# richarddurbin/modimizer

Measured on AMD Instinct MI355X. Metric: Gbp/s hashed+sketched (k=21,d=64), higher is better.
Workload: dtype u64; 1 GPU; BASELINE config 2: 10 Gbp synthetic ONT-like reads (log-normal N50 20 kb, 5% subs, 30x of a 333 Mbp genome), k=21 d=64 seed=17, seqhash scan + modset build (table bits 30); reads_per_gpu=598835, bases_per_gpu=10000000000, modimizers_per_gpu=156043826, modset_entries=102967436, k=21, d=64, table_bits=30, parallelism=reads sharded x1, modset per GPU

## Files before the change

modimizer_amd/csrc/mg_bucket.hip:

```cpp
#include "mg_table.h"



template <bool PACKED>
__device__ __forceinline__ void mgOccurrence (const MgBucketArgs &a, U32 b, U64 x, U32 t, U64 *m, U32 *ord)
{
  if (PACKED)
    { *ord = (U32) (x & (((U64) 1 << a.f.ordBits) - 1));
      *m = ((U64) (b >> a.f.loB) << a.f.remBits) | (x >> a.f.ordBits);
    }
  else { *m = x; *ord = t; }
}

__device__ __forceinline__ void mgDedupCount (const MgBucketArgs &a, U32 *sOrd, U32 *sCnt, U32 at, U32 ord)
{
  const U32 tok = mgToken (ord);
  if (a.markDup)
    { const U32 old = atomicMax (&sOrd[at], tok);
      const U32 loser = old > tok ? tok : old;
      if (loser MG_ABLATE_AND (!(a.debug & 1))) a.flags[0x7fffffffu - loser] = 0;
    }
  else atomicMax (&sOrd[at], tok);
  atomicAdd (&sCnt[at], 1u);
}
// ... 189 lines not shown
  const U32 R = a.g.R, T = blockDim.x, tid = threadIdx.x;
  unsigned long long *sKey = reinterpret_cast<unsigned long long *> (mgDynLds);
  U32 *sOrd = reinterpret_cast<U32 *> (mgDynLds + (size_t) R * 8);
  U32 *sCnt = sOrd + R;
  U32 *sGrp = sCnt + R;
  const U32 nGrp = a.nSlices + 1;
  U32 b = blockIdx.x * bucketsPerBlock, bEnd = b + bucketsPerBlock;
  U64 hotAt = blockIdx.x; const U64 nHot = HOT ? a.hotCount[1] : 0;
  if (HOT) { if (hotAt >= nHot) return; }
  else
    { if (bEnd > a.nBuckets) bEnd = a.nBuckets;
      if (b >= bEnd) return;
    }
  for (U32 i = tid ; i < R ; i += T) { sKey[i] = 0; sOrd[i] = 0; sCnt[i] = 0; }
  if (tid < MG_RANK_GROUPS) sGrp[tid] = 0;
  for ( ; ; )
  {
  if (HOT) { b = a.hotBuckets[hotAt]; bEnd = b + 1; }
  U64 lo = a.bucketStart[b], hi = a.bucketStart[b + 1];
  U32 occNow = a.occ[b];
  U64 ck[MG_BUCKET_PREFETCH]; U32 ct[MG_BUCKET_PREFETCH];
#pragma unroll
  for (int j = 0 ; j < MG_BUCKET_PREFETCH ; ++j)
    { U64 i = lo + (U64) j * T + tid; ck[j] = 0; ct[j] = 0; if (!HOT && i < hi) { ck[j] = __builtin_nontemporal_load (&a.pK[i]); if (!PACKED) ct[j] = __builtin_nontemporal_load (&a.pT[i]); } }
  __syncthreads ();
  for ( ; b < bEnd ; ++b)
    {
      U64 nlo = hi, nhi = hi;
      U64 nk[MG_BUCKET_PREFETCH]; U32 nt[MG_BUCKET_PREFETCH];
#pragma unroll
// ... 47 lines not shown
              rk[j] = 0; rc[j] = 0; ro[j] = 0; rp[j] = 0;
              if (i < R) rk[j] = sKey[i];
              if (rk[j])
                { rc[j] = sCnt[i]; ro[j] = sOrd[i];
                  sKey[i] = 0; sOrd[i] = 0; sCnt[i] = 0;
                  rk[j] = (rk[j] - 1) | (SLOT ? (unsigned long long) i << MG_SLOT_SHIFT : 0ull);
                  if (rc[j]) rp[j] = atomicAdd (&sGrp[mgIsAssigned (ro[j]) ? a.nSlices : ((0x7fffffffu - ro[j]) >> a.sliceShift)], 1u);
                }
            }
          __syncthreads ();
          const int lane = (int) (tid & 63);
          const U32 gv = (U32) lane < nGrp ? sGrp[lane] : 0;
          const U32 gIncl = mgWaveInclusiveSum (gv);
          const U32 gBase = gIncl - gv;
          const U32 total = (U32) __builtin_amdgcn_readlane ((int) gIncl, 63);
          if (tid < 64)
            { if ((U32) lane <= nGrp) a.sliceOff[(U64) b * (nGrp + 1) + lane] = (unsigned short) gBase;
              if (lane == 0) a.uniqCount[b] = total;
            }
#pragma unroll
          for (int j = 0 ; j < PER ; ++j)
            { const U32 grp = mgIsAssigned (ro[j]) ? a.nSlices : ((0x7fffffffu - ro[j]) >> a.sliceShift);
              const U32 at = (U32) __shfl ((int) gBase, (int) (rc[j] ? grp : 0)) + rp[j];
              if (rc[j]) { sKey[at] = rk[j]; sOrd[at] = ro[j]; sCnt[at] = rc[j]; }
            }
          __syncthreads ();
          if (tid < MG_RANK_GROUPS) sGrp[tid] = 0;
          for (U32 i = tid ; i < total ; i += T)
            { const U64 k = sKey[i]; const U32 ord = sOrd[i], c = sCnt[i];
              sKey[i] = 0; sOrd[i] = 0; sCnt[i] = 0;
              if (true MG_ABLATE_AND (!(a.debug & 8)))
                { __builtin_nontemporal_store (k, &a.pK[lo + i]); __builtin_nontemporal_store (ord, &a.pT[lo + i]); __builtin_nontemporal_store (c, &a.pC[lo + i]); }
              if (!a.markDup && !mgIsAssigned (ord) MG_ABLATE_AND (!(a.debug & 1))) a.flags[0x7fffffffu - ord] = 1;
            }
          __syncthreads ();
        }
      lo = nlo; hi = nhi; occNow = occNext;
#pragma unroll
      for (int j = 0 ; j < MG_BUCKET_PREFETCH ; ++j) { ck[j] = nk[j]; ct[j] = nt[j]; }
    }
  if (!HOT) break;
  hotAt += gridDim.x;
  if (hotAt >= nHot) break;
  }
}

__device__ __forceinline__ U32 mgPlaceStarts (U32 *cnt, unsigned short *sStart, int *sWave, U32 R, U32 T, U32 tid, U32 n)
{
  const U32 per = (R + 4 * T - 1) / (4 * T) * 4;
  const U32 j0 = tid * per, j1 = j0 + per < R ? j0 + per : R;
  U32 vS = 0; int vM = 0;
  for (U32 j = j0 ; j < j1 ; j += 4)
    { const uint4 c = *reinterpret_cast<const uint4 *> (&cnt[j]);
      int m = (int) j - (int) vS;               vM = m > vM ? m : vM; vS += c.x;
      m = (int) (j + 1) - (int) vS;             vM = m > vM ? m : vM; vS += c.y;
      m = (int) (j + 2) - (int) vS;             vM = m > vM ? m : vM; vS += c.z;
      m = (int) (j + 3) - (int) vS;             vM = m > vM ? m : vM; vS += c.w;
    }
  const int lane = (int) (tid & 63);
// ... 245 lines not shown
{
  unsigned long long sum = 0; U32 mx = 0;
  for (U32 b = blockIdx.x * 256 + threadIdx.x ; b < nBuckets ; b += gridDim.x * 256) { const U32 c = uniqCount[b]; sum += c; mx = c > mx ? c : mx; }
  sum = mgWaveReduce<MgSum> ((U64) sum); mx = mgWaveReduce<MgMax> (mx);
  if ((threadIdx.x & 63) == 0) { if (sum) atomicAdd (&out[0], sum); if (mx) atomicMax (&out[1], (unsigned long long) mx); }
}


MgStatus mgBucketDedup (const MgBucketArgs &a, bool packed, unsigned threads, unsigned grid, U32 perBlock, size_t lds, hipStream_t st)
{
  const U32 R = a.g.R;
  const bool bigR = R > MG_DEDUP_PER * 1024u;
  if (R > MG_DEDUP_PER_BIG * 1024u) { mgSetError ("internal: bucket of %u slots", R); return MG_ERR_ARG; }
  if ((U64) threads * (bigR ? MG_DEDUP_PER_BIG : MG_DEDUP_PER) < R)
    { mgSetError ("internal: %u threads for a bucket of %u slots", threads, R); return MG_ERR_ARG; }
  MG_HIP (hipMemsetAsync (a.hotCount, 0, 16, st));
  MG_LAUNCH (MG_K_HOT_REDUCE, st, mgHotPlanKernel, dim3 ((a.nBuckets + 255) / 256), dim3 (256), 0, st, a);
  const size_t ldsHot = (size_t) R * 16 + 16;
  const MgStatus s = mgForFlag (packed, [&] (auto PK) -> MgStatus
    { if (ldsHot > 48 * 1024) MG_HIP (hipFuncSetAttribute ((const void *) mgHotReduceKernel<decltype (PK)::value>, hipFuncAttributeMaxDynamicSharedMemorySize, (int) ldsHot));
      MG_LAUNCH (MG_K_HOT_REDUCE, st, mgHotReduceKernel<decltype (PK)::value>, dim3 (1024), dim3 (threads), ldsHot, st, a);
      return MG_OK;
    });
  if (s) return s;
  return mgForFlag (packed, [&] (auto PK) -> MgStatus { return mgForFlag (a.slotShift != 0, [&] (auto SL) -> MgStatus { return mgForFlag (bigR, [&] (auto BIG) -> MgStatus
    { constexpr bool pk = decltype (PK)::value, sl = decltype (SL)::value;
      constexpr int per = decltype (BIG)::value ? MG_DEDUP_PER_BIG : MG_DEDUP_PER;
      if (lds > 48 * 1024)
        { MG_HIP (hipFuncSetAttribute ((const void *) mgBucketDedupKernel<pk, sl, per, false>, hipFuncAttributeMaxDynamicSharedMemorySize, (int) lds));
          MG_HIP (hipFuncSetAttribute ((const void *) mgBucketDedupKernel<pk, sl, per, true>, hipFuncAttributeMaxDynamicSharedMemorySize, (int) lds));
        }
// ... 32 lines not shown
```

modimizer_amd/csrc/mg_common.h:

```cpp
#ifndef MG_COMMON_H
#define MG_COMMON_H
#include "mg_knobs.h"

#include <hip/hip_runtime.h>
#include <stdint.h>
#include <time.h>
#include <algorithm>
#include <vector>
#include "modgpu.h"

#define MG_WAVE 64

#define MG_SCAN_THREADS   256
#define MG_POS_PER_THREAD 64
#define MG_TILE_BASES     (64 * MG_POS_PER_THREAD)
#define MG_TILE_WORDS     (MG_TILE_BASES / 16)

struct MgHashParams {
  U64 factor1;
  U64 mask;
  int k;
  int shift1;
  U32 d;
  int dShift;
// ... 189 lines not shown
  U16 *baseDepth;
  bool baseZero;
  U64 *liveHist;
  bool liveHistValid;
  U32 size;
  U32 max;
  U32 syncedMax;
  U64 *counters;
  bool pendingDepth;
  bool dirty;
  U64 *find8;
  U64 find8Cap;
  U64 find8Version, version;
  bool empty;
  U64 *pin;
  int newPct;
  int loadPct;
  int  maxLog2Slots;
  U32  wantR;
  U64  diag[7];
  int  tightPct;
};
MgStatus mgTableAlloc (MgTable *t, U64 slotsWanted, hipStream_t st);
MgStatus mgTableEnsure (MgTable *t, U64 nIncoming, hipStream_t st);
MgStatus mgTableRollback (MgTable *t, hipStream_t st);
MgStatus mgTableClean (MgTable *t, hipStream_t st);
void     mgTableForget (MgTable *t, hipStream_t st);
size_t   mgTableAddScratchBytes (const MgTable *t, U64 n);
bool     mgTableUseBuckets (const MgTable *t, U64 n);
MgStatus mgTableAdd (MgTable *t, const U64 *dKmer, U64 n, int withDepth, void *scratch, hipStream_t st,
// ... 32 lines not shown
```

modimizer_amd/csrc/mg_knobs.c:

```c
#define _GNU_SOURCE
#include <pthread.h>
#include <sched.h>
#include <stdio.h>
#include <stdlib.h>
#include <string.h>
#include <unistd.h>
#include <sys/mman.h>
#include "mg_knobs.h"

static MgKnobs gKnobs;
static pthread_once_t gOnce = PTHREAD_ONCE_INIT;

static long num (const char *name)
{ const char *e = getenv (name); return e && *e ? atol (e) : MG_KNOB_UNSET; }

static void readAll (void)
{
  MgKnobs k;
  const char *e = getenv ("MODGPU_TABLE_PATH");
  k.tablePath = e && *e ? (long) e[0] : MG_KNOB_UNSET;
  e = getenv ("MODGPU_FIND_PATH");
  k.findPath = e && *e ? (long) e[0] : MG_KNOB_UNSET;
  k.partPacked = num ("MODGPU_PART_PACKED");       k.partBig = num ("MODGPU_PART_BIG");
  k.addChunk = num ("MODGPU_ADD_CHUNK");           k.scanGrid = num ("MODGPU_SCAN_GRID");
  k.scanGeneric = num ("MODGPU_SCAN_GENERIC");     k.scanHist = num ("MODGPU_SCAN_HIST");
  k.scanDiv64 = num ("MODGPU_SCAN_DIV64");        k.minTiled = num ("MODGPU_MIN_TILED");
  k.minTile = num ("MODGPU_MIN_TILE");
  k.noSegmentInput = num ("MODGPU_NO_SEGMENT_INPUT");
  k.rankSliceShift = num ("MODGPU_RANK_SLICE_SHIFT");
  k.flagPolarity = num ("MODGPU_FLAG_POLARITY");   k.mergeSlots = num ("MODGPU_MERGE_SLOTS");
  k.mergePlace = num ("MODGPU_MERGE_PLACE");
  k.bucketR = num ("MODGPU_BUCKET_R");             k.bucketT = num ("MODGPU_BUCKET_T");
  e = getenv ("MODGPU_HOT_SPLIT");
  k.hotSplit = e && *e ? atol (e) : MG_KNOB_UNSET;
  { const char *c = e ? strchr (e, ',') : 0; k.hotChunk = c ? atol (c + 1) : MG_KNOB_UNSET; }
  k.noAvx2 = num ("MODGPU_NO_AVX2");               k.textHost = num ("MODGPU_TEXT_HOST");
  k.textWindowKb = num ("MODGPU_TEXT_WINDOW_KB");   k.bgzfHost = num ("MODGPU_BGZF_HOST");
// ... 61 lines not shown
```

modimizer_amd/csrc/mg_knobs.h:

```cpp
#ifndef MG_KNOBS_H
#define MG_KNOBS_H
#include <limits.h>
#ifdef __cplusplus
extern "C" {
#endif
#define MG_KNOB_UNSET LONG_MIN
typedef struct {
  long findPath;
  long tablePath;
  long partPacked;
  long partBig;
  long addChunk;
  long scanGrid;
  long scanGeneric;
  long minTile;
  long minTiled;
  long scanDiv64;
  long scanHist;
  long noSegmentInput;
  long rankSliceShift;
  long flagPolarity;
  long mergeSlots;
  long mergePlace;
  long bucketR, bucketT;
  long hotSplit, hotChunk;
  long noAvx2;
  long textHost;
  long textWindowKb;
  long fileBatchMbp;
  long fileBatchBases;
  long readsetHost;
  long overlapCands;
  long testModsBatch;
  long overlapLds;
  long bgzfHost;
  long textIdsDevice;
  long gzipHost;
  long gzipChunkKb;
  long gzipBatch;
  long gzipRatio;
// ... 32 lines not shown
```

modimizer_amd/csrc/mg_modsetdev.hip:

```cpp
#include <unordered_map>
#include "mg_api_int.h"
#include "mg_xfer.h"

struct MgOnDevice
{ int before = -1; bool moved = false;
  explicit MgOnDevice (int dev) { if (dev >= 0 && hipGetDevice (&before) == hipSuccess && before != dev) moved = hipSetDevice (dev) == hipSuccess; }
  ~MgOnDevice () { if (moved) (void) hipSetDevice (before); }
};

static std::mutex gRegLock;
static std::unordered_map<const Modset *, MgDev *> gReg;
extern "C" { volatile int mgLiveDeviceModsets = 0; }

MgDev *mgDevLookup (const Modset *ms)
{ std::lock_guard<std::mutex> g (gRegLock); auto it = gReg.find (ms); return it == gReg.end () ? 0 : it->second; }

static void mgDevFree (MgDev *d)
{
  if (!d) return;
  MgOnDevice here (d->device);
  if (d->hPin) (void) hipHostFree (d->hPin);
  if (d->built)
    { (void) hipFree (d->t.slots); (void) hipFree (d->t.value); (void) hipFree (d->t.occ); (void) hipFree (d->t.find8);
      (void) hipFree (d->t.baseDepth); (void) hipFree (d->t.counters); (void) hipFree (d->t.liveHist);
    }
  if (d->side) { (void) hipStreamSynchronize (d->side); (void) hipStreamDestroy (d->side); }
  d->arena.release (); d->arena2.release ();
  for (int i = 0 ; i < 2 ; ++i) if (d->scanned[i]) (void) hipEventDestroy (d->scanned[i]);
  if (d->inputReady) (void) hipEventDestroy (d->inputReady);
  delete d;
}

static void mgDevDrop (Modset *ms, MgDev *d)
{
  { std::lock_guard<std::mutex> g (gRegLock); gReg.erase (ms); mgLiveDeviceModsets = (int) gReg.size (); }
  mgDevFree (d);
}

static MgStatus mgDevOnCallersGpu (const MgDev *d, bool quiet = false)
// ... 16 lines not shown
  MgTable &t = d->t;
  if (ms->tableBits < 20 || ms->tableBits > 32)
    { mgSetError ("device modset supports table bits 20..32 (got %d)", ms->tableBits); return MG_ERR_ARG; }
  memset (&t, 0, sizeof (t));
  t.maxLog2Slots = ms->tableBits - 1;
  t.kbits = 2 * ms->hasher->k;
  t.wantR = 4096;
  { const long r = mgKnobs ()->bucketR; if (r != MG_KNOB_UNSET && r >= 256) t.wantR = (U32) r; }
  t.size = ms->size;
  t.pin = d->hPin + 24;
  U64 cap = (ms->tableSize >> 2);
  MG_HIP (hipMalloc ((void **) &t.value, cap * sizeof (U64)));
  MG_HIP (hipMalloc ((void **) &t.baseDepth, cap * sizeof (U16)));
  MG_HIP (hipMalloc ((void **) &t.counters, 64));
  d->built = true;
  MG_HIP (hipMemsetAsync (t.baseDepth, 0, cap * sizeof (U16), st));
  MG_HIP (hipMemsetAsync (t.counters, 0, 64, st));
  { MgStatus s0 = mgTableEnsure (&t, ms->max, st); if (s0) return s0; }
  t.max = 0; t.syncedMax = 0;
  t.baseZero = !ms->max;
  if (ms->max)
    { MG_HIP (hipStreamSynchronize (st));
      MgStatus s;
      if ((s = mgXferH2D (t.value, ms->value, ((size_t) ms->max + 1) * sizeof (U64)))) return s;
      if ((s = mgXferH2D (t.baseDepth, ms->depth, ((size_t) ms->max + 1) * sizeof (U16)))) return s;
      if ((s = mgTableLoadHost (&t, t.value, 1, ms->max, st))) return s;
      MG_HIP (hipStreamSynchronize (st));
      t.max = t.syncedMax = ms->max;
    }
  d->hostIndexMax = ms->max;
// ... 194 lines not shown


U64 mgAddChunkSize (void)
{
  const long c = mgKnobs ()->addChunk;
  U64 v = c != MG_KNOB_UNSET && c > 0 ? (U64) c : ((U64) 1 << 30);
  if (v > ((U64) 1 << 30)) v = (U64) 1 << 30;
  return v;
}

static MgStatus mgAddChunk (Modset *ms, MgDev *d, const U64 *dKmer, U64 n, U32 *dIndexOut, int withDepth,
                            void *scratch, hipStream_t st, const MgHistReq *counted = 0, const MgSegSrc *segSrc = 0)
{
  MgTable &t = d->t;
  MgStatus s;
  MG_HIP (hipMemsetAsync (t.counters, 0, 16, st));
  if ((s = mgTableAdd (&t, dKmer, n, withDepth, scratch, st, counted, segSrc))) return s;
  volatile U64 *c = d->hPin;
  MG_HIP (hipMemcpyAsync (d->hPin, t.counters, 16, hipMemcpyDeviceToHost, st));
  MG_HIP (hipStreamSynchronize (st));
  U64 newMax = (U64) t.max + c[0];
  if (c[1] || newMax >= t.size)
    {
      if ((s = mgTableRollback (&t, st))) return s;
      mgSetError ("hashTableSize %u is too small for %llu", t.size, (unsigned long long) newMax);
      return MG_ERR_CAPACITY;
    }
  t.max = (U32) newMax;
  ms->max = t.max;
  if (n >= 4096) t.newPct = (int) (c[0] * 100 / n);
  if (dIndexOut && (s = mgTableFind (&t, dKmer, n, dIndexOut, st))) return s;
// ... 145 lines not shown
```

modimizer_amd/csrc/mg_part.hip:

```cpp
#include "mg_table.h"


__global__ void mgSubSegKernel (const MgSegSrc src, U64 n, U32 sub, MgSubSeg *__restrict__ subSeg)
{
  const U64 q = (U64) blockIdx.x * blockDim.x + threadIdx.x;
  if (q * sub >= n) return;
  const U32 w = mgSegOfOrdinal (src, q * sub);
  MgSubSeg e; e.w = w; e.s0 = src.segStart[w]; e.s1 = src.segStart[w + 1];
  subSeg[q] = e;
}

__global__ __launch_bounds__ (MG_PART_MAXBINS)
void mgPartChunksKernel (const U64 *__restrict__ segStart, U32 nSeg, U32 chunkElems, U32 *__restrict__ chunkBase)
{
  __shared__ U32 sS[MG_PART_MAXBINS];
  const U32 t = threadIdx.x;
  U32 c = t < nSeg ? (U32) ((segStart[t + 1] - segStart[t] + chunkElems - 1) / chunkElems) : 0;
  sS[t] = c;
  __syncthreads ();
  for (int off = 1 ; off < MG_PART_MAXBINS ; off <<= 1)
    { U32 v = t >= (U32) off ? sS[t - off] : 0;
      __syncthreads ();
      sS[t] += v;
      __syncthreads ();
// ... 252 lines not shown
      c = nc; seg = nseg; lo = nlo; hi = nhi; sub = nsub; have = nhave;
    }
}


MgStatus mgPartPass (const MgTable *t, MgPartPassArgs &p, hipStream_t st)
{
  MgGeom g = mgGeomOf (t);
  MgSegSrc src = {};
  if (p.inMode == MG_EL_SEG)
    { if (!p.segSrc || !p.subSeg || !p.counted) { mgSetError ("internal: segment input needs its counts"); return MG_ERR_ARG; }
      src = *p.segSrc;
      const U64 nSub = (p.n + MG_PART_SUB - 1) / MG_PART_SUB;
      MG_LAUNCH (MG_K_PART, st, mgSubSegKernel, dim3 ((unsigned) ((nSub + 255) / 256)), dim3 (256), 0, st, src, p.n, (U32) MG_PART_SUB, p.subSeg);
    }
  if (p.counted) MG_HIP (hipMemcpy2DAsync (p.binCount, sizeof (U32), p.counted, MG_HIST_STRIDE * sizeof (U32), sizeof (U32), p.nBins, hipMemcpyDeviceToDevice, st));
  else MG_HIP (hipMemsetAsync (p.binCount, 0, (size_t) p.nSeg * p.nBins * sizeof (U32), st));
  const int bigEnv = mgKnobs ()->partBig == MG_KNOB_UNSET ? 1 : (int) mgKnobs ()->partBig;
  const bool big = bigEnv && p.packed && p.nBins <= MG_PART_BIG_BINS && MG_PART_THREADS == 1024;
  p.subElems = (U32) (big ? MG_PART_SUB_BIG : MG_PART_SUB);
  const U32 chunkElems = 2u * p.subElems;
  MG_LAUNCH (MG_K_PART, st, mgPartChunksKernel, dim3 (1), dim3 (MG_PART_MAXBINS), 0, st, p.segStart, p.nSeg, chunkElems, p.chunkBase);
  const unsigned maxChunks = p.maxChunks = (unsigned) (p.n / chunkElems + p.nSeg + 1);
  const int sgEnv = mgKnobs ()->scatterGrid == MG_KNOB_UNSET ? 0 : (int) mgKnobs ()->scatterGrid;
  unsigned scatterGrid = maxChunks < (unsigned) (sgEnv > 0 ? sgEnv : 1024) ? maxChunks : (unsigned) (sgEnv > 0 ? sgEnv : 1024);
  const dim3 hg (maxChunks < 4096 ? maxChunks : 4096), sg (scatterGrid);
  if (!p.counted && p.digitIn)
    MG_LAUNCH (MG_K_PART_HIST, st, mgPartHistBytesKernel, hg, dim3 (256), 0, st, p.digitIn, p.nBins, p.segStart, p.chunkBase, p.nSeg, chunkElems, p.binCount);
  else if (!p.counted)
    {
#define MG_HIST(IN) MG_LAUNCH (MG_K_PART_HIST, st, mgPartHistKernel<IN>, hg, dim3 (256), 0, st, p.kIn, g, p.f, p.shift, p.nBins, p.segStart, p.chunkBase, p.nSeg, chunkElems, p.binCount)
// ... 19 lines not shown
```

modimizer_amd/csrc/mg_scan.hip:

```cpp
#include <stdlib.h>
#include <atomic>
#include "mg_prefix.h"


__global__ void mgPackKernel (const U8 *__restrict__ bases, U64 nBases, U32 *__restrict__ words, U64 nWords)
{
  U64 i = (U64) blockIdx.x * blockDim.x + threadIdx.x;
  U64 stride = (U64) gridDim.x * blockDim.x;
  const bool aligned = (((uintptr_t) bases) & 15) == 0;
  for ( ; i < nWords ; i += stride)
    { U64 b0 = i * 16;
      U32 w = 0;
      if (b0 + 16 <= nBases && aligned)
        { uint4 v = *reinterpret_cast<const uint4 *> (bases + b0);
          U32 q[4] = { v.x, v.y, v.z, v.w };
#pragma unroll
          for (int j = 0 ; j < 4 ; ++j)
            { U32 x = q[j];
              U32 n = ((x & 3) << 6) | (((x >> 8) & 3) << 4) | (((x >> 16) & 3) << 2) | ((x >> 24) & 3);
              w |= n << (24 - 8 * j);
            }
        }
      else if (b0 < nBases)
        { for (int j = 0 ; j < 16 && b0 + j < nBases ; ++j)
// ... 476 lines not shown
    }
  if (threadIdx.x == 0) o.out[0] = total;
  __threadfence_system ();
  __syncthreads ();
  if (threadIdx.x == 0) __hip_atomic_store (const_cast<U64 *> (o.flag), o.seq, __ATOMIC_RELEASE, __HIP_MEMORY_SCOPE_SYSTEM);
}

__global__ __launch_bounds__ (1024)
void mgSegScanKernel (const U64 *__restrict__ blockCount, U32 nBlocks, U64 segCap, U64 capacity,
                      U64 *__restrict__ segStart, U64 *__restrict__ dCount)
{
  __shared__ U64 sV[8192 + 1024];
  __shared__ U64 sWaveSum[16], sWaveMax[16];
  const int tid = threadIdx.x, lane = tid & 63, wave = tid >> 6;
  U64 carry = 0, gmx = 0;
  for (U32 base = 0 ; base < nBlocks ; base += 8192)
    {
#pragma unroll
      for (int j = 0 ; j < 8 ; ++j)
        { U32 e = (U32) j * 1024 + tid, b = base + e;
          sV[e + (e >> 3)] = b < nBlocks ? blockCount[b] : 0;
        }
      __syncthreads ();
      U64 c[8], sum = 0, mx = 0;
#pragma unroll
      for (int j = 0 ; j < 8 ; ++j) { c[j] = sV[tid * 9 + j]; sum += c[j]; if (c[j] > mx) mx = c[j]; }
      U64 incl = sum, wmx = mx;
#pragma unroll
      for (int off = 1 ; off < 64 ; off <<= 1)
        { U32 lo = __shfl_up ((U32) incl, off), hi = __shfl_up ((U32) (incl >> 32), off);
          if (lane >= off) incl += ((U64) hi << 32) | lo;
          U32 ml = __shfl_xor ((U32) wmx, off), mh = __shfl_xor ((U32) (wmx >> 32), off);
          U64 o = ((U64) mh << 32) | ml; if (o > wmx) wmx = o;
        }
      if (lane == 63) { sWaveSum[wave] = incl; sWaveMax[wave] = wmx; }
      __syncthreads ();
// ... 275 lines not shown
```

modimizer_amd/csrc/mg_table.h:

```cpp
#ifndef MG_TABLE_H
#define MG_TABLE_H
#include <stdlib.h>
#include <string.h>
#include "mg_prefix.h"

#define MG_ASSIGNED 0x80000000u
#define MG_R_QUANTUM 64u
#ifdef MG_BUILD_PRIO
#define MG_BUILD_PRIO() __builtin_amdgcn_s_setprio (3)
#else
#define MG_BUILD_PRIO() do { } while (0)
#endif
#ifdef MG_ABLATE
#define MG_ABLATE_AND(x) && (x)
#else
#define MG_ABLATE_AND(x)
#endif
__device__ __forceinline__ U32 mgToken (U64 o) { return 0x7fffffffu - (U32) o; }
__device__ __forceinline__ bool mgIsAssigned (U32 v) { return (v & MG_ASSIGNED) != 0; }
__device__ __forceinline__ U64 mgKeyOf (const uint4 &v) { return ((U64) v.y << 32) | v.x; }
__device__ __forceinline__ U32 mgIndexOf (U32 ordWord) { return mgIsAssigned (ordWord) ? (ordWord & ~MG_ASSIGNED) : 0; }
__device__ __forceinline__ bool mgLiveEntry (const uint4 &v, U32 keepMax) { return (v.x | v.y) && mgIsAssigned (v.z) && (v.z & ~MG_ASSIGNED) <= keepMax; }


// ... 64 lines not shown

#ifndef MG_PART_THREADS
#define MG_PART_THREADS 1024
#endif
#define MG_PART_SUB_BIG (2 * MG_PART_SUB)
#define MG_PART_BIG_BINS 256

struct MgPartPassArgs {
  int inMode; bool packed; MgPartFmt f;
  const U64 *kIn; const U32 *tIn; U64 n;
  const U64 *segStart; U32 nSeg;
  int shift; U32 nBins;
  U64 *kOut; U32 *tOut; U64 *binStart;
  unsigned long long *cursor; U32 *binCount, *chunkBase;
  const U32 *counted;
  const MgSegSrc *segSrc; MgSubSeg *subSeg;
  unsigned long long *runTab; int runMode;
  unsigned char *digitOut; int nextShift; U32 nextBins;
  const unsigned char *digitIn;
  U32 subElems, maxChunks;
};
MgStatus mgPartPass (const MgTable *t, MgPartPassArgs &p, hipStream_t st);

struct MgBucketArgs {
  MgSlot *slots; MgGeom g; U32 nBuckets;
  const U64 *bucketStart;
  U64 *pK; U32 *pT; U32 *pC;
  MgPartFmt f;
  U32 *uniqCount;
  U32 *occ;
// ... 80 lines not shown
```

modimizer_amd/csrc/mg_table.hip:

```cpp
#include "mg_table.h"


__global__ void mgTableInsertKernel (MgSlot *__restrict__ slots, MgGeom g, const U64 *__restrict__ kmer, U64 n,
                                     U32 *__restrict__ slotId, int withDepth, U64 *counters)
{
  U64 o = (U64) blockIdx.x * blockDim.x + threadIdx.x;
  const U64 stride = (U64) gridDim.x * blockDim.x;
  for ( ; o < n ; o += stride)
    { const U64 m = mgMixK (kmer[o], g.kbits), key = m + 1;
      const U64 base = (U64) mgBucketOfM (m, g) * g.R;
      U32 at = mgHomeOfM (m, g);
      bool ok = false;
      for (U32 probes = 0 ; probes < g.R ; ++probes)
        { U64 cur = slots[base + at].key;
          if (cur == 0)
            { cur = atomicCAS ((unsigned long long *) &slots[base + at].key, 0ull, (unsigned long long) key);
              if (cur == 0) cur = key;
            }
          if (cur == key) { ok = true; break; }
          at = mgNextSlot (at, g.R);
        }
      if (!ok) { counters[1] = 1; slotId[o] = 0xffffffffu; continue; }
      const U64 s = base + at;
      U32 v = slots[s].ord;
// ... 670 lines not shown
                                 U64 *unitCount, U64 *unitBase, const U32 *slotId, MgRankGrp *grp, hipStream_t st)
{
  const MgSegSrc noSrc = {};
  U32 nBlocks; const U64 rows = mgRankRowsPerUnit (n, &nBlocks);
  MG_LAUNCH (MG_K_RANK_COUNT, st, mgRankCountKernel, dim3 (nBlocks), dim3 (256), 0, st, flags, n, rows, unitCount);
  MG_LAUNCH (MG_K_RANK_SCAN, st, (mgGroupSumKernel<U64, U64>), dim3 (1), dim3 (MG_GROUP_THREADS), 0, st, unitCount, unitBase, nBlocks * 4, t->counters);
#define MG_ASSIGN(DIRECT, SEG, KMER, SRC, SUB) MG_LAUNCH (MG_K_TABLE_ASSIGN, st, (mgRankAssignKernel<DIRECT, SEG>), dim3 (nBlocks), dim3 (256), 0, st, \
                                                          flags, KMER, SRC, SUB, n, rows, unitBase, t->max, t->size, t->value, t->slots, slotId, grp)
  if (slotId) MG_ASSIGN (true, false, dKmer, noSrc, (const MgSubSeg *) 0);
  else if (segSrc) MG_ASSIGN (false, true, (const U64 *) 0, *segSrc, subSeg);
  else MG_ASSIGN (false, false, dKmer, noSrc, (const MgSubSeg *) 0);
#undef MG_ASSIGN
  return MG_OK;
}

static MgStatus mgAddTighten (MgTable *t, int tightPct, const U32 *uniqCount, U64 *fullest, hipStream_t st)
{
  const U64 NB = (U64) 1 << t->log2NB;
  { MgStatus s = mgUniqStats (uniqCount, (U32) NB, (unsigned long long *) (t->counters + 2), st); if (s) return s; }
  MG_HIP (hipMemcpyAsync (t->pin, t->counters + 1, 24, hipMemcpyDeviceToHost, st));
  MG_HIP (hipStreamSynchronize (st));
  const U64 over = t->pin[0], U = t->pin[1], M = t->pin[2];
  if (over) return MG_OK;
  *fullest = M;
  U64 Rn = (U * 100 / ((U64) NB * (U64) tightPct) + 1 + MG_R_QUANTUM - 1) / MG_R_QUANTUM * MG_R_QUANTUM;
  const U64 Rfit = (M + M / 8 + 16 + MG_R_QUANTUM - 1) / MG_R_QUANTUM * MG_R_QUANTUM;
  if (Rn < Rfit) Rn = Rfit;
  if (Rn < MG_TIGHT_MIN_R) Rn = MG_TIGHT_MIN_R;
  if (Rn < t->R) { t->R = (U32) Rn; t->nSlots = (U64) NB * Rn; }
  return MG_OK;
}

size_t mgTableAddScratchBytes (const MgTable *t, U64 n)
{
  (void) t;
  U64 NB = (U64) 1 << 18;
  size_t rank = mgAl256 (n)  + 2 * mgAl256 ((MG_RANK_UNITS + 8) * 8) + mgAl256 ((n / 64 + 2) * sizeof (MgRankGrp));
  size_t direct = mgAl256 (n * 4);
  size_t part = 2 * (mgAl256 (n * 8) + mgAl256 (n * 4)) + mgAl256 (n * 4)
              + mgAl256 ((NB + 2) * 8) * 3 + mgAl256 ((NB + 2) * 4) * 2 + mgAl256 (((U64) MG_PART_MAXBINS + 2) * 8) * 3 + 2 * mgAl256 ((U64) MG_PART_MAXBINS * 16 * 8 + 4096)
              + mgAl256 ((MG_PART_MAXBINS + 2) * 4) + mgAl256 ((MG_PART_MAXBINS + 2 + n / MG_PART_CHUNK + MG_PART_MAXBINS + 2) * 4)
              + mgAl256 ((size_t) (MG_RANK_GROUPS + 2) * NB * sizeof (unsigned short)) + mgAl256 ((n / MG_PART_SUB + 2) * 24)
              + mgAl256 (mgHotItemsCap (n) * 8) + mgAl256 (mgHotItemsCap (n) * 4) + 256;
  return rank + (direct > part ? direct : part) + 4096;
}

MgStatus mgTableAdd (MgTable *t, const U64 *dKmer, U64 n, int withDepth, void *scratch, hipStream_t st,
                     const MgHistReq *counted, const MgSegSrc *segSrc)
{
  if (!n) return MG_OK;
  if (segSrc && !mgTableAddTakesSegments (t, n, counted)) { mgSetError ("internal: this insert needs the dense k-mers"); return MG_ERR_ARG; }
  t->liveHistValid = false;
  if (withDepth) t->pendingDepth = true;
  const bool wasEmpty = t->empty && t->max == 0;
  t->empty = false; ++t->version;
  MgGeom g = mgGeomOf (t);
  char *wb = (char *) scratch;
  unsigned char *flags = (unsigned char *) wb;       wb += mgAl256 (n);
  U64 *blockCount = (U64 *) wb;                      wb += mgAl256 ((MG_RANK_UNITS + 8) * 8);
  U64 *blockBase = (U64 *) wb;                       wb += mgAl256 ((MG_RANK_UNITS + 8) * 8);
  MgRankGrp *grp = (MgRankGrp *) wb;                 wb += mgAl256 ((n / 64 + 2) * sizeof (MgRankGrp));
  MG_HIP (hipMemsetAsync (blockCount, 0, (MG_RANK_UNITS + 8) * 8, st));

  if (!mgTableUseBuckets (t, n))
    { U32 *slotId = (U32 *) wb;
      { MgStatus cs = mgTableClean (t, st); if (cs) return cs; }
      MG_LAUNCH (MG_K_TABLE_INSERT, st, mgTableInsertKernel, dim3 (mgGridWide (n)), dim3 (256), 0, st, t->slots, g, dKmer, n, slotId, withDepth, t->counters);
      MG_LAUNCH (MG_K_TABLE_FLAG, st, mgDirectFlagKernel, dim3 (mgGridWide (n)), dim3 (256), 0, st, t->slots, slotId, n, flags);
      { MgStatus as = mgAssignIndices (t, flags, dKmer, (const MgSegSrc *) 0, (const MgSubSeg *) 0, n, blockCount, blockBase, slotId, grp, st); if (as) return as; }
      MG_HIP (hipGetLastError ());
      return mgTableMarkOccupied (t, dKmer, n, st);
    }

  const U64 NB = (U64) 1 << t->log2NB;
  U64 *kA = (U64 *) wb;  wb += mgAl256 (n * 8);
  U32 *tA = (U32 *) wb;  wb += mgAl256 (n * 4);
  U64 *kB = (U64 *) wb;  wb += mgAl256 (n * 8);
  U32 *tB = (U32 *) wb;  wb += mgAl256 (n * 4);
  U32 *cB = (U32 *) wb;  wb += mgAl256 (n * 4);
  U64 *fineStart = (U64 *) wb;                wb += mgAl256 ((NB + 2) * 8);
// ... 4 lines not shown
  U64 *coarseStart = (U64 *) wb;              wb += mgAl256 (((U64) MG_PART_MAXBINS + 2) * 8);
  unsigned long long *coarseCursor = (unsigned long long *) wb; wb += mgAl256 (((U64) MG_PART_MAXBINS + 2) * 8 * 16);
  U64 *whole = (U64 *) wb;                    wb += mgAl256 (((U64) MG_PART_MAXBINS + 2) * 8);
  U32 *coarseCount = (U32 *) wb;              wb += mgAl256 ((MG_PART_MAXBINS + 2) * 4);
  U32 *chunkBase = (U32 *) wb;                wb += mgAl256 ((MG_PART_MAXBINS + 2 + n / MG_PART_CHUNK + MG_PART_MAXBINS + 2) * 4);
  unsigned short *sliceOff = (unsigned short *) wb;   wb += mgAl256 ((size_t) (MG_RANK_GROUPS + 2) * NB * sizeof (unsigned short));
  MgSubSeg *subSeg = (MgSubSeg *) wb;         wb += mgAl256 ((n / MG_PART_SUB + 2) * sizeof (MgSubSeg));
  U64 *hotItems = (U64 *) wb;                 wb += mgAl256 (mgHotItemsCap (n) * 8);
  U32 *hotBuckets = (U32 *) wb;               wb += mgAl256 (mgHotItemsCap (n) * 4);
  unsigned long long *hotCount = (unsigned long long *) wb; wb += 256;

  MgAddPlan plan;
  mgAddPlan (t, n, wasEmpty, &plan);
  const int hiB = plan.hiB, loB = plan.loB;
  const U32 *pre = (counted && counted->binCount && counted->log2NB == t->log2NB && counted->kbits == t->kbits && !counted->hiB) ? counted->binCount : 0;
  U64 segInit[2] = { 0, n };
  MG_HIP (hipMemcpyAsync (whole, segInit, 16, hipMemcpyHostToDevice, st));
  MgStatus s;
  MgPartPassArgs p1 = {};
  p1.inMode = segSrc ? MG_EL_SEG : MG_EL_DENSE; p1.packed = plan.packed; p1.f = plan.f; p1.kIn = dKmer; p1.n = n; p1.segStart = whole; p1.nSeg = 1;
  p1.nBins = (U32) 1 << hiB; p1.chunkBase = chunkBase; p1.counted = pre; p1.segSrc = segSrc; p1.subSeg = subSeg;
  if (!loB)
    { p1.kOut = kB; p1.tOut = tB; p1.binStart = fineStart; p1.cursor = fineCursor; p1.binCount = fineCount;
      if ((s = mgPartPass (t, p1, st))) return s;
    }
  else
    {
      unsigned char *digits = plan.digitBytes ? reinterpret_cast<unsigned char *> (cB) : 0;
      p1.shift = loB; p1.kOut = kA; p1.tOut = tA; p1.binStart = coarseStart; p1.cursor = coarseCursor; p1.binCount = coarseCount;
      p1.digitOut = digits; p1.nextBins = (U32) 1 << loB;
      if ((s = mgPartPass (t, p1, st))) return s;
      MgPartPassArgs p2 = {};
      p2.inMode = plan.packed ? MG_EL_PACKED : MG_EL_WIDE; p2.packed = plan.packed; p2.f = plan.f; p2.kIn = kA; p2.tIn = tA; p2.n = n; p2.segStart = coarseStart; p2.nSeg = (U32) 1 << hiB;
      p2.nBins = (U32) 1 << loB; p2.kOut = kB; p2.tOut = tB; p2.binStart = fineStart; p2.cursor = fineCursor; p2.binCount = fineCount; p2.chunkBase = chunkBase;
      p2.digitIn = digits;
      if ((s = mgPartPass (t, p2, st))) return s;
    }

  MG_HIP (hipMemsetAsync (flags, plan.markDup ? 1 : 0, n, st));
  MgBucketArgs a;
  a.slots = t->slots; a.g = g; a.nBuckets = (U32) NB; a.bucketStart = fineStart;
  a.pK = kB; a.pT = tB; a.pC = cB; a.uniqCount = uniqCount; a.occ = t->occ; a.flags = flags;
  a.grp = grp; a.baseMax = t->max; a.size = t->size; a.withDepth = withDepth;
  a.markDup = plan.markDup; a.slotShift = plan.slotShift; a.place = plan.place;
  a.sliceShift = plan.sliceShift; a.nSlices = plan.nSlices; a.sliceOff = sliceOff;
  a.hotSplit = plan.hotSplit; a.hotChunk = plan.hotChunk; a.hotItems = hotItems; a.hotCount = hotCount; a.hotBuckets = hotBuckets;
  a.counters = t->counters; a.f = plan.f;
#ifdef MG_ABLATE
  { const long dbg = mgKnobs ()->bucketDebug; a.debug = dbg != MG_KNOB_UNSET ? (int) dbg : 0; }
#endif
  const bool track = t->max == 0 && t->baseZero;
  a.liveHist = 0;
  if (track)
    { if (!t->liveHist) MG_HIP (hipMalloc ((void **) &t->liveHist, 65536 * sizeof (U64)));
      MG_HIP (hipMemsetAsync (t->liveHist, 0, 65536 * sizeof (U64), st));
      a.liveHist = (unsigned long long *) t->liveHist;
    }
  t->liveHistValid = track;
  size_t lds = mgMergeLdsBytes (t->R);
  { const size_t ldsDedup = (size_t) t->R * 16 + MG_RANK_GROUPS * 4; if (ldsDedup > lds) lds = ldsDedup; }
  const int bThreadsEnv = mgKnobs ()->bucketT == MG_KNOB_UNSET ? 0 : (int) mgKnobs ()->bucketT;
  const unsigned bThreads = mgBucketThreads (t->R, bThreadsEnv);
  U32 perBlock;
  const unsigned bGrid = mgBucketGrid (NB, &perBlock);

  if ((s = mgBucketDedup (a, plan.packed, bThreads, bGrid, perBlock, lds, st))) return s;
  U64 fullest = t->R;
  if (plan.tighten)
    { if ((s = mgAddTighten (t, plan.tightPct, uniqCount, &fullest, st))) return s;
      if (t->R != a.g.R) { a.g = mgGeomOf (t); lds = mgMergeLdsBytes (t->R); }
    }
  if ((s = mgAssignIndices (t, flags, dKmer, segSrc, subSeg, n, blockCount, blockBase, (const U32 *) 0, grp, st))) return s;
  if ((s = mgRankLookup (a, st))) return s;
  if ((s = mgBucketMerge (a, fullest, bThreads, bGrid, perBlock, lds, st))) return s;
  MG_HIP (hipGetLastError ());
  return MG_OK;
}

__global__ void mgMarkOccKernel (MgGeom g, const U64 *__restrict__ kmer, U64 n, U32 *__restrict__ occ)
{
  U64 o = (U64) blockIdx.x * blockDim.x + threadIdx.x;
  const U64 stride = (U64) gridDim.x * blockDim.x;
  for ( ; o < n ; o += stride)
    { U32 b = mgBucketOfM (mgMixK (kmer[o], g.kbits), g);
      if (!occ[b]) occ[b] = 1;
    }
}

// ... 200 lines not shown
```

Before: 1236 Gbp/s.

## Fold add-path memsets into one preset kernel and overlap tighten readback

```diff
diff --git a/modimizer_amd/csrc/mg_bucket.hip b/modimizer_amd/csrc/mg_bucket.hip
--- a/modimizer_amd/csrc/mg_bucket.hip
+++ b/modimizer_amd/csrc/mg_bucket.hip
@@ -227,6 +227,7 @@
     }
   for (U32 i = tid ; i < R ; i += T) { sKey[i] = 0; sOrd[i] = 0; sCnt[i] = 0; }
   if (tid < MG_RANK_GROUPS) sGrp[tid] = 0;
+  U32 uSum = 0, uMax = 0;
   for ( ; ; )
   {
   if (HOT) { b = a.hotBuckets[hotAt]; bEnd = b + 1; }
@@ -304,6 +305,7 @@
           const U32 gIncl = mgWaveInclusiveSum (gv);
           const U32 gBase = gIncl - gv;
           const U32 total = (U32) __builtin_amdgcn_readlane ((int) gIncl, 63);
+          uSum += total; uMax = total > uMax ? total : uMax;
           if (tid < 64)
             { if ((U32) lane <= nGrp) a.sliceOff[(U64) b * (nGrp + 1) + lane] = (unsigned short) gBase;
               if (lane == 0) a.uniqCount[b] = total;
@@ -333,6 +335,10 @@
   hotAt += gridDim.x;
   if (hotAt >= nHot) break;
   }
+  if (tid == 0 && uSum)
+    { atomicAdd (reinterpret_cast<unsigned long long *> (&a.counters[2]), (unsigned long long) uSum);
+      atomicMax (reinterpret_cast<unsigned long long *> (&a.counters[3]), (unsigned long long) uMax);
+    }
 }
 
 __device__ __forceinline__ U32 mgPlaceStarts (U32 *cnt, unsigned short *sStart, int *sWave, U32 R, U32 T, U32 tid, U32 n)
@@ -608,7 +614,6 @@
   if (R > MG_DEDUP_PER_BIG * 1024u) { mgSetError ("internal: bucket of %u slots", R); return MG_ERR_ARG; }
   if ((U64) threads * (bigR ? MG_DEDUP_PER_BIG : MG_DEDUP_PER) < R)
     { mgSetError ("internal: %u threads for a bucket of %u slots", threads, R); return MG_ERR_ARG; }
-  MG_HIP (hipMemsetAsync (a.hotCount, 0, 16, st));
   MG_LAUNCH (MG_K_HOT_REDUCE, st, mgHotPlanKernel, dim3 ((a.nBuckets + 255) / 256), dim3 (256), 0, st, a);
   const size_t ldsHot = (size_t) R * 16 + 16;
   const MgStatus s = mgForFlag (packed, [&] (auto PK) -> MgStatus
diff --git a/modimizer_amd/csrc/mg_common.h b/modimizer_amd/csrc/mg_common.h
--- a/modimizer_amd/csrc/mg_common.h
+++ b/modimizer_amd/csrc/mg_common.h
@@ -227,6 +227,7 @@
   U64 find8Version, version;
   bool empty;
   U64 *pin;
+  hipEvent_t tightDone;
   int newPct;
   int loadPct;
   int  maxLog2Slots;
diff --git a/modimizer_amd/csrc/mg_knobs.c b/modimizer_amd/csrc/mg_knobs.c
--- a/modimizer_amd/csrc/mg_knobs.c
+++ b/modimizer_amd/csrc/mg_knobs.c
@@ -21,6 +21,8 @@
   k.tablePath = e && *e ? (long) e[0] : MG_KNOB_UNSET;
   e = getenv ("MODGPU_FIND_PATH");
   k.findPath = e && *e ? (long) e[0] : MG_KNOB_UNSET;
+  e = getenv ("MODGPU_UNIQ_STATS");
+  k.uniqStats = e && *e ? (long) e[0] : MG_KNOB_UNSET;
   k.partPacked = num ("MODGPU_PART_PACKED");       k.partBig = num ("MODGPU_PART_BIG");
   k.addChunk = num ("MODGPU_ADD_CHUNK");           k.scanGrid = num ("MODGPU_SCAN_GRID");
   k.scanGeneric = num ("MODGPU_SCAN_GENERIC");     k.scanHist = num ("MODGPU_SCAN_HIST");
diff --git a/modimizer_amd/csrc/mg_knobs.h b/modimizer_amd/csrc/mg_knobs.h
--- a/modimizer_amd/csrc/mg_knobs.h
+++ b/modimizer_amd/csrc/mg_knobs.h
@@ -24,6 +24,7 @@
   long mergePlace;
   long bucketR, bucketT;
   long hotSplit, hotChunk;
+  long uniqStats;
   long noAvx2;
   long textHost;
   long textWindowKb;
diff --git a/modimizer_amd/csrc/mg_modsetdev.hip b/modimizer_amd/csrc/mg_modsetdev.hip
--- a/modimizer_amd/csrc/mg_modsetdev.hip
+++ b/modimizer_amd/csrc/mg_modsetdev.hip
@@ -23,6 +23,7 @@
   if (d->built)
     { (void) hipFree (d->t.slots); (void) hipFree (d->t.value); (void) hipFree (d->t.occ); (void) hipFree (d->t.find8);
       (void) hipFree (d->t.baseDepth); (void) hipFree (d->t.counters); (void) hipFree (d->t.liveHist);
+      if (d->t.tightDone) (void) hipEventDestroy (d->t.tightDone);
     }
   if (d->side) { (void) hipStreamSynchronize (d->side); (void) hipStreamDestroy (d->side); }
   d->arena.release (); d->arena2.release ();
@@ -69,6 +70,7 @@
   MG_HIP (hipMalloc ((void **) &t.baseDepth, cap * sizeof (U16)));
   MG_HIP (hipMalloc ((void **) &t.counters, 64));
   d->built = true;
+  MG_HIP (hipEventCreateWithFlags (&t.tightDone, hipEventDisableTiming));
   MG_HIP (hipMemsetAsync (t.baseDepth, 0, cap * sizeof (U16), st));
   MG_HIP (hipMemsetAsync (t.counters, 0, 64, st));
   { MgStatus s0 = mgTableEnsure (&t, ms->max, st); if (s0) return s0; }
@@ -293,7 +295,6 @@
 {
   MgTable &t = d->t;
   MgStatus s;
-  MG_HIP (hipMemsetAsync (t.counters, 0, 16, st));
   if ((s = mgTableAdd (&t, dKmer, n, withDepth, scratch, st, counted, segSrc))) return s;
   volatile U64 *c = d->hPin;
   MG_HIP (hipMemcpyAsync (d->hPin, t.counters, 16, hipMemcpyDeviceToHost, st));
diff --git a/modimizer_amd/csrc/mg_part.hip b/modimizer_amd/csrc/mg_part.hip
--- a/modimizer_amd/csrc/mg_part.hip
+++ b/modimizer_amd/csrc/mg_part.hip
@@ -290,7 +290,8 @@
       const U64 nSub = (p.n + MG_PART_SUB - 1) / MG_PART_SUB;
       MG_LAUNCH (MG_K_PART, st, mgSubSegKernel, dim3 ((unsigned) ((nSub + 255) / 256)), dim3 (256), 0, st, src, p.n, (U32) MG_PART_SUB, p.subSeg);
     }
-  if (p.counted) MG_HIP (hipMemcpy2DAsync (p.binCount, sizeof (U32), p.counted, MG_HIST_STRIDE * sizeof (U32), sizeof (U32), p.nBins, hipMemcpyDeviceToDevice, st));
+  if (p.counted && p.countsSet) { }
+  else if (p.counted) MG_HIP (hipMemcpy2DAsync (p.binCount, sizeof (U32), p.counted, MG_HIST_STRIDE * sizeof (U32), sizeof (U32), p.nBins, hipMemcpyDeviceToDevice, st));
   else MG_HIP (hipMemsetAsync (p.binCount, 0, (size_t) p.nSeg * p.nBins * sizeof (U32), st));
   const int bigEnv = mgKnobs ()->partBig == MG_KNOB_UNSET ? 1 : (int) mgKnobs ()->partBig;
   const bool big = bigEnv && p.packed && p.nBins <= MG_PART_BIG_BINS && MG_PART_THREADS == 1024;
diff --git a/modimizer_amd/csrc/mg_scan.hip b/modimizer_amd/csrc/mg_scan.hip
--- a/modimizer_amd/csrc/mg_scan.hip
+++ b/modimizer_amd/csrc/mg_scan.hip
@@ -514,12 +514,17 @@
   __shared__ U64 sWaveSum[16], sWaveMax[16];
   const int tid = threadIdx.x, lane = tid & 63, wave = tid >> 6;
   U64 carry = 0, gmx = 0;
+  U64 pre[8];
+#pragma unroll
+  for (int j = 0 ; j < 8 ; ++j) { const U32 b = (U32) j * 1024 + tid; pre[j] = b < nBlocks ? blockCount[b] : 0; }
   for (U32 base = 0 ; base < nBlocks ; base += 8192)
     {
 #pragma unroll
-      for (int j = 0 ; j < 8 ; ++j)
-        { U32 e = (U32) j * 1024 + tid, b = base + e;
-          sV[e + (e >> 3)] = b < nBlocks ? blockCount[b] : 0;
+      for (int j = 0 ; j < 8 ; ++j) { const U32 e = (U32) j * 1024 + tid; sV[e + (e >> 3)] = pre[j]; }
+      if (base + 8192 < nBlocks)
+        {
+#pragma unroll
+          for (int j = 0 ; j < 8 ; ++j) { const U32 b = base + 8192 + (U32) j * 1024 + tid; pre[j] = b < nBlocks ? blockCount[b] : 0; }
         }
       __syncthreads ();
       U64 c[8], sum = 0, mx = 0;
diff --git a/modimizer_amd/csrc/mg_table.h b/modimizer_amd/csrc/mg_table.h
--- a/modimizer_amd/csrc/mg_table.h
+++ b/modimizer_amd/csrc/mg_table.h
@@ -102,6 +102,7 @@
   U64 *kOut; U32 *tOut; U64 *binStart;
   unsigned long long *cursor; U32 *binCount, *chunkBase;
   const U32 *counted;
+  bool countsSet;
   const MgSegSrc *segSrc; MgSubSeg *subSeg;
   unsigned long long *runTab; int runMode;
   unsigned char *digitOut; int nextShift; U32 nextBins;
diff --git a/modimizer_amd/csrc/mg_table.hip b/modimizer_amd/csrc/mg_table.hip
--- a/modimizer_amd/csrc/mg_table.hip
+++ b/modimizer_amd/csrc/mg_table.hip
@@ -708,12 +708,19 @@
   return MG_OK;
 }
 
-static MgStatus mgAddTighten (MgTable *t, int tightPct, const U32 *uniqCount, U64 *fullest, hipStream_t st)
+static MgStatus mgAddTightenAsk (MgTable *t, const U32 *uniqCount, hipStream_t st)
+{
+  if (mgKnobs ()->uniqStats == 'k')
+    { MgStatus s = mgUniqStats (uniqCount, (U32) 1 << t->log2NB, (unsigned long long *) (t->counters + 2), st); if (s) return s; }
+  MG_HIP (hipMemcpyAsync (t->pin, t->counters + 1, 24, hipMemcpyDeviceToHost, st));
+  if (t->tightDone) MG_HIP (hipEventRecord (t->tightDone, st));
+  return MG_OK;
+}
+static MgStatus mgAddTighten (MgTable *t, int tightPct, U64 *fullest, hipStream_t st)
 {
   const U64 NB = (U64) 1 << t->log2NB;
-  { MgStatus s = mgUniqStats (uniqCount, (U32) NB, (unsigned long long *) (t->counters + 2), st); if (s) return s; }
-  MG_HIP (hipMemcpyAsync (t->pin, t->counters + 1, 24, hipMemcpyDeviceToHost, st));
-  MG_HIP (hipStreamSynchronize (st));
+  if (t->tightDone) MG_HIP (hipEventSynchronize (t->tightDone));
+  else MG_HIP (hipStreamSynchronize (st));
   const U64 over = t->pin[0], U = t->pin[1], M = t->pin[2];
   if (over) return MG_OK;
   *fullest = M;
@@ -723,6 +730,25 @@
   if (Rn < MG_TIGHT_MIN_R) Rn = MG_TIGHT_MIN_R;
   if (Rn < t->R) { t->R = (U32) Rn; t->nSlots = (U64) NB * Rn; }
   return MG_OK;
+}
+
+struct MgAddPreset {
+  U64 *counters;
+  U64 *blockCount; U32 nBlockCount;
+  unsigned long long *hotCount, *liveHist;
+  U64 *whole; U64 n;
+  const U32 *counted; U32 *binCount; U32 nBins;
+};
+#define MG_PRESET_GRID 64
+__global__ __launch_bounds__ (256)
+void mgAddPresetKernel (const MgAddPreset p)
+{
+  const U64 tid = (U64) blockIdx.x * 256 + threadIdx.x, stride = (U64) gridDim.x * 256;
+  for (U64 i = tid ; i < p.nBlockCount ; i += stride) p.blockCount[i] = 0;
+  if (p.liveHist) for (U64 i = tid ; i < 65536 ; i += stride) p.liveHist[i] = 0;
+  if (tid < 4) p.counters[tid] = 0;
+  if (tid == 0) { p.hotCount[0] = 0; p.hotCount[1] = 0; p.whole[0] = 0; p.whole[1] = p.n; }
+  if (p.counted) for (U64 i = tid ; i < p.nBins ; i += stride) p.binCount[i] = p.counted[i * MG_HIST_STRIDE];
 }
 
 size_t mgTableAddScratchBytes (const MgTable *t, U64 n)
@@ -742,7 +768,7 @@
 MgStatus mgTableAdd (MgTable *t, const U64 *dKmer, U64 n, int withDepth, void *scratch, hipStream_t st,
                      const MgHistReq *counted, const MgSegSrc *segSrc)
 {
-  if (!n) return MG_OK;
+  if (!n) { MG_HIP (hipMemsetAsync (t->counters, 0, 32, st)); return MG_OK; }
   if (segSrc && !mgTableAddTakesSegments (t, n, counted)) { mgSetError ("internal: this insert needs the dense k-mers"); return MG_ERR_ARG; }
   t->liveHistValid = false;
   if (withDepth) t->pendingDepth = true;
@@ -754,10 +780,11 @@
   U64 *blockCount = (U64 *) wb;                      wb += mgAl256 ((MG_RANK_UNITS + 8) * 8);
   U64 *blockBase = (U64 *) wb;                       wb += mgAl256 ((MG_RANK_UNITS + 8) * 8);
   MgRankGrp *grp = (MgRankGrp *) wb;                 wb += mgAl256 ((n / 64 + 2) * sizeof (MgRankGrp));
-  MG_HIP (hipMemsetAsync (blockCount, 0, (MG_RANK_UNITS + 8) * 8, st));
 
   if (!mgTableUseBuckets (t, n))
     { U32 *slotId = (U32 *) wb;
+      MG_HIP (hipMemsetAsync (t->counters, 0, 32, st));
+      MG_HIP (hipMemsetAsync (blockCount, 0, (MG_RANK_UNITS + 8) * 8, st));
       { MgStatus cs = mgTableClean (t, st); if (cs) return cs; }
       MG_LAUNCH (MG_K_TABLE_INSERT, st, mgTableInsertKernel, dim3 (mgGridWide (n)), dim3 (256), 0, st, t->slots, g, dKmer, n, slotId, withDepth, t->counters);
       MG_LAUNCH (MG_K_TABLE_FLAG, st, mgDirectFlagKernel, dim3 (mgGridWide (n)), dim3 (256), 0, st, t->slots, slotId, n, flags);
@@ -792,12 +819,17 @@
   mgAddPlan (t, n, wasEmpty, &plan);
   const int hiB = plan.hiB, loB = plan.loB;
   const U32 *pre = (counted && counted->binCount && counted->log2NB == t->log2NB && counted->kbits == t->kbits && !counted->hiB) ? counted->binCount : 0;
-  U64 segInit[2] = { 0, n };
-  MG_HIP (hipMemcpyAsync (whole, segInit, 16, hipMemcpyHostToDevice, st));
+  const bool track = t->max == 0 && t->baseZero;
+  if (track && !t->liveHist) MG_HIP (hipMalloc ((void **) &t->liveHist, 65536 * sizeof (U64)));
+  { MgAddPreset ps;
+    ps.counters = t->counters; ps.blockCount = blockCount; ps.nBlockCount = MG_RANK_UNITS + 8; ps.hotCount = hotCount; ps.liveHist = track ? (unsigned long long *) t->liveHist : 0;
+    ps.whole = whole; ps.n = n; ps.counted = pre; ps.binCount = loB ? coarseCount : fineCount; ps.nBins = (U32) 1 << hiB;
+    MG_LAUNCH (MG_K_MEMSET, st, mgAddPresetKernel, dim3 (MG_PRESET_GRID), dim3 (256), 0, st, ps);
+  }
   MgStatus s;
   MgPartPassArgs p1 = {};
   p1.inMode = segSrc ? MG_EL_SEG : MG_EL_DENSE; p1.packed = plan.packed; p1.f = plan.f; p1.kIn = dKmer; p1.n = n; p1.segStart = whole; p1.nSeg = 1;
-  p1.nBins = (U32) 1 << hiB; p1.chunkBase = chunkBase; p1.counted = pre; p1.segSrc = segSrc; p1.subSeg = subSeg;
+  p1.nBins = (U32) 1 << hiB; p1.chunkBase = chunkBase; p1.counted = pre; p1.countsSet = pre != 0; p1.segSrc = segSrc; p1.subSeg = subSeg;
   if (!loB)
     { p1.kOut = kB; p1.tOut = tB; p1.binStart = fineStart; p1.cursor = fineCursor; p1.binCount = fineCount;
       if ((s = mgPartPass (t, p1, st))) return s;
@@ -827,13 +859,7 @@
 #ifdef MG_ABLATE
   { const long dbg = mgKnobs ()->bucketDebug; a.debug = dbg != MG_KNOB_UNSET ? (int) dbg : 0; }
 #endif
-  const bool track = t->max == 0 && t->baseZero;
-  a.liveHist = 0;
-  if (track)
-    { if (!t->liveHist) MG_HIP (hipMalloc ((void **) &t->liveHist, 65536 * sizeof (U64)));
-      MG_HIP (hipMemsetAsync (t->liveHist, 0, 65536 * sizeof (U64), st));
-      a.liveHist = (unsigned long long *) t->liveHist;
-    }
+  a.liveHist = track ? (unsigned long long *) t->liveHist : 0;
   t->liveHistValid = track;
   size_t lds = mgMergeLdsBytes (t->R);
   { const size_t ldsDedup = (size_t) t->R * 16 + MG_RANK_GROUPS * 4; if (ldsDedup > lds) lds = ldsDedup; }
@@ -844,12 +870,13 @@
 
   if ((s = mgBucketDedup (a, plan.packed, bThreads, bGrid, perBlock, lds, st))) return s;
   U64 fullest = t->R;
+  if (plan.tighten && (s = mgAddTightenAsk (t, uniqCount, st))) return s;
+  if ((s = mgAssignIndices (t, flags, dKmer, segSrc, subSeg, n, blockCount, blockBase, (const U32 *) 0, grp, st)) || (s = mgRankLookup (a, st)))
+    { (void) hipStreamSynchronize (st); return s; }
   if (plan.tighten)
-    { if ((s = mgAddTighten (t, plan.tightPct, uniqCount, &fullest, st))) return s;
+    { if ((s = mgAddTighten (t, plan.tightPct, &fullest, st))) { (void) hipStreamSynchronize (st); return s; }
       if (t->R != a.g.R) { a.g = mgGeomOf (t); lds = mgMergeLdsBytes (t->R); }
     }
-  if ((s = mgAssignIndices (t, flags, dKmer, segSrc, subSeg, n, blockCount, blockBase, (const U32 *) 0, grp, st))) return s;
-  if ((s = mgRankLookup (a, st))) return s;
   if ((s = mgBucketMerge (a, fullest, bThreads, bGrid, perBlock, lds, st))) return s;
   MG_HIP (hipGetLastError ());
   return MG_OK;
```

Result: no change. 1244 Gbp/s, median of 6 (+0.7%).
